# chrischoy/DeepGlobalRegistration

Measured on NVIDIA H100. Metric: scan_pairs_per_sec, higher is better.
Workload: dtype f32

## Files before the change

### deepglobalregistration_b200/csrc/spconv_ring.h

```cpp
#pragma once

#if defined(__CUDACC__)
#define DGR_RING_HD __host__ __device__ __forceinline__
#else
#define DGR_RING_HD inline
#endif

namespace spconv_ring {

constexpr int kStages = 2;
constexpr int kIdxSlots = kStages + 1;
constexpr int kMaxRun = 8;

DGR_RING_HD int stage_of(unsigned g) { return (int)(g % kStages); }
DGR_RING_HD unsigned full_parity(unsigned g) { return (g / kStages) & 1u; }
DGR_RING_HD unsigned empty_parity(unsigned g) { return (g / kStages - 1u) & 1u; }
DGR_RING_HD int idx_slot(unsigned tile) { return (int)(tile % kIdxSlots); }

constexpr int kMinWaves = 2;
DGR_RING_HD int tile_run(int n_tiles, int resident) {
  const int r = n_tiles / (kMinWaves * (resident > 0 ? resident : 1));
  return r < 1 ? 1 : (r > kMaxRun ? kMaxRun : r);
}

}
```

### deepglobalregistration_b200/csrc/spconv_tc.cu

```cuda
#include <stdlib.h>

#include "common.cuh"
#include "spconv_ring.h"
#include "tc_common.cuh"

namespace {

using namespace tc;
using namespace spconv_ring;

#define DGR_TRY_RC(expr)             \
  do {                              \
    int32_t rc__ = (expr);          \
    if (rc__ != DGR_OK) return rc__; \
  } while (0)

constexpr int kConsumerWarps = 8;
constexpr int kProducerThreads = 128;
constexpr int kThreadsTC = kConsumerWarps * 32 + kProducerThreads;
constexpr int kTileM = 128;
constexpr int kChunk = 32;
constexpr int kATileBytes = kTileM * 128;
constexpr int kGatherRows = kTileM / (kProducerThreads / 8);
static_assert(kMaxRun <= 32, "one warp lists the tiles of a run");

struct TileDesc {
  int kappa, p0, rows;
};

struct TcShared {
  unsigned long long full[kStages];
  unsigned long long empty[kStages];
  int n_run;
  TileDesc tiles[kMaxRun];
  int out_rows[kIdxSlots][kTileM];
};

constexpr bool tc_line_epilogue(int nt) { return nt >= 128; }
constexpr int kScratchLd = 40;
constexpr int kScratchBytes = 16 * kScratchLd * 4;

constexpr size_t tc_smem_bytes(int nt) {
  return sizeof(TcShared) + 1024 + (size_t)kStages * (2 * kATileBytes + 2 * nt * 128) +
         (tc_line_epilogue(nt) ? (size_t)kConsumerWarps * kScratchBytes : 0);
}

constexpr int tc_min_ctas(int nt, bool f16) { return nt >= 128 || f16 ? 1 : 2; }
constexpr int kProducerRegs = 104, kConsumerRegs = 200;

template <int NT, bool kF16, int kPasses>
__global__ void __launch_bounds__(kThreadsTC, tc_min_ctas(NT, kF16))
spconv_tc_kernel(const float* __restrict__ in_feat, int cin, const unsigned char* __restrict__ wt, int cout,
                 const int32_t* __restrict__ in_idx, const int32_t* __restrict__ out_idx,
                 const int32_t* __restrict__ kofs, const int32_t* __restrict__ tile_k,
                 const int32_t* __restrict__ tile_start, int n_tiles, int run, const float* __restrict__ amax_in,
                 const float* __restrict__ w_inv_scale, float* __restrict__ out) {
  constexpr int kCh = kF16 ? 64 : kChunk;
  constexpr int kV = kF16 ? 2 : 1;
  constexpr int kBatches = kV, kBatchRows = kGatherRows / kBatches;
  constexpr int kBTileBytes = NT * 128;
  constexpr int kStageBytes = 2 * kATileBytes + 2 * kBTileBytes;
  extern __shared__ __align__(16) unsigned char smem_dyn[];
  TcShared& sh = *reinterpret_cast<TcShared*>(smem_dyn);
  unsigned char* stage0 = reinterpret_cast<unsigned char*>(
      (reinterpret_cast<uintptr_t>(smem_dyn) + sizeof(TcShared) + 1023) & ~(uintptr_t)1023);
  const int t = threadIdx.x, warp = __shfl_sync(0xffffffffu, t >> 5, 0), lane = t & 31;
  const int n_chunks = cin / kCh;
  const uint32_t b_tile_bytes = (uint32_t)cout * 128;
  const uint32_t slab_bytes = 2 * b_tile_bytes;
  const uint32_t full0 = smem_u32(&sh.full[0]), empty0 = smem_u32(&sh.empty[0]);

  if (t == 0) {
    for (int s = 0; s < kStages; ++s) {
      mbar_init(full0 + 8 * s, kProducerThreads + 1);
      mbar_init(empty0 + 8 * s, kConsumerWarps);
    }
    asm volatile("fence.mbarrier_init.release.cluster;" ::: "memory");
  }
  if (NT > cout) {
    const int pad_pieces = (NT - cout) * 8;
    for (int i = t; i < kStages * 2 * pad_pieces; i += kThreadsTC) {
      const int tile = i / pad_pieces, e = i % pad_pieces;
      *reinterpret_cast<uint4*>(stage0 + (tile >> 1) * kStageBytes + 2 * kATileBytes + (tile & 1) * kBTileBytes +
                                (cout + (e >> 3)) * 128 + (e & 7) * 16) = make_uint4(0u, 0u, 0u, 0u);
    }
  }
  if (warp == 0) {
    const int tile = blockIdx.x * run + lane;
    TileDesc d = {0, 0, 0};
    if (lane < run && tile < n_tiles) {
      d.kappa = tile_k[tile];
      d.p0 = tile_start[tile];
      d.rows = min(kTileM, kofs[d.kappa + 1] - d.p0);
    }
    const unsigned live = __ballot_sync(0xffffffffu, d.rows > 0);
    if (d.rows > 0) sh.tiles[__popc(live & ((1u << lane) - 1u))] = d;
    if (lane == 0) sh.n_run = __popc(live);
  }
  __syncthreads();
  const int n_run = sh.n_run;
  if (n_run == 0) return;

  if (warp >= kConsumerWarps) {
    if (NT >= 128) asm volatile("setmaxnreg.dec.sync.aligned.u32 %0;" ::"n"(kProducerRegs));
    const int pt = t - kConsumerWarps * 32, piece = pt & 7, rgrp = pt >> 3;
    const uint32_t a_off = (uint32_t)(rgrp * 128 + ((piece ^ (rgrp & 7)) << 4));
    const float sx = kF16 ? f16_scale_for(__ldg(amax_in)) : 1.f;
    auto load_idx = [&](int ti, int (&src)[kGatherRows], int& oj) {
      const TileDesc d = sh.tiles[ti < n_run ? ti : 0];
      const int rows = ti < n_run ? d.rows : 0;
#pragma unroll
      for (int i = 0; i < kGatherRows; ++i) {
        const int r = i * 16 + rgrp;
        src[i] = r < rows ? __ldg(in_idx + d.p0 + r) : -1;
      }
      oj = pt < rows ? __ldg(out_idx + d.p0 + pt) : -1;
    };
    int src[kGatherRows], src_next[kGatherRows], oj, oj_next;
    float4 v[kBatchRows][kV];
    auto load_a = [&](int c, int h) {
#pragma unroll
      for (int i = 0; i < kBatchRows; ++i)
#pragma unroll
        for (int u = 0; u < kV; ++u) {
          const int row = src[h * kBatchRows + i];
          v[i][u] = row >= 0 ? __ldg(reinterpret_cast<const float4*>(in_feat + (size_t)row * cin + c * kCh +
                                                                      piece * (4 * kV) + 4 * u))
                             : make_float4(0.f, 0.f, 0.f, 0.f);
        }
    };
    load_idx(0, src, oj);
    load_idx(1, src_next, oj_next);
    load_a(0, 0);
    unsigned g = 0;
    for (int ti = 0; ti < n_run; ++ti) {
      const unsigned char* slab = wt + (size_t)sh.tiles[ti].kappa * n_chunks * slab_bytes;
      for (int c = 0; c < n_chunks; ++c, ++g) {
        const int s = stage_of(g);
        unsigned char* a_hi = stage0 + (size_t)s * kStageBytes;
        unsigned char* a_lo = a_hi + kATileBytes;
        unsigned char* b_hi = a_lo + kATileBytes;
        if (g >= kStages) mbar_wait(empty0 + 8 * s, empty_parity(g));
        if (pt == 0) {
          const unsigned char* bsrc = slab + (size_t)c * slab_bytes;
          mbar_arrive_expect_tx(full0 + 8 * s, kPasses == 3 ? slab_bytes : b_tile_bytes);
          bulk_g2s(smem_u32(b_hi), bsrc, b_tile_bytes, full0 + 8 * s);
          if (kPasses == 3) bulk_g2s(smem_u32(b_hi + kBTileBytes), bsrc + b_tile_bytes, b_tile_bytes, full0 + 8 * s);
        }
        if (c == 0) sh.out_rows[idx_slot(ti)][pt] = oj;
#pragma unroll
        for (int h = 0; h < kBatches; ++h) {
#pragma unroll
          for (int i = 0; i < kBatchRows; ++i) {
            const uint32_t off = a_off + (h * kBatchRows + i) * 2048;
            if (kF16) split_store_f16(v[i][0], v[i][kV - 1], sx, a_hi, a_lo, off);
            else split_store(v[i][0], a_hi, a_lo, off);
          }
          if (h + 1 < kBatches) {
            load_a(c, h + 1);
          } else if (c + 1 < n_chunks) {
            load_a(c + 1, 0);
          } else if (ti + 1 < n_run) {
#pragma unroll
            for (int i = 0; i < kGatherRows; ++i) src[i] = src_next[i];
            oj = oj_next;
            load_a(0, 0);
            load_idx(ti + 2, src_next, oj_next);
          }
        }
        fence_proxy_async();
        mbar_arrive(full0 + 8 * s);
      }
    }
    return;
  }

  if (NT >= 128) asm volatile("setmaxnreg.inc.sync.aligned.u32 %0;" ::"n"(kConsumerRegs));
  const int wg = warp >> 2;
  const int r0 = wg * 64 + (warp & 3) * 16 + (lane >> 2);
  const float inv = kF16 ? __ldg(w_inv_scale) / f16_scale_for(__ldg(amax_in)) : 1.f;
  auto release = [&](unsigned gq) {
    __syncwarp();
    if (lane == 0) mbar_arrive(empty0 + 8 * stage_of(gq));
  };
  unsigned g = 0;
  for (int ti = 0; ti < n_run; ++ti) {
    float acc[NT / 2];
#pragma unroll
    for (int i = 0; i < NT / 2; ++i) acc[i] = 0.f;
    for (int c = 0; c < n_chunks; ++c, ++g) {
      const uint32_t a_hi = smem_u32(stage0 + (size_t)stage_of(g) * kStageBytes);
      const uint32_t b_hi = a_hi + 2 * kATileBytes;
      mbar_wait(full0 + 8 * stage_of(g), full_parity(g));
      wgmma_fence();
      const uint32_t a0 = a_hi + wg * (kATileBytes / 2);
      mma_chunk<NT, kF16, kPasses>(acc, a0, a0 + kATileBytes, b_hi, b_hi + kBTileBytes);
      wgmma_commit();
      wgmma_wait<1>();
      if (c > 0) release(g - 1);
    }
    wgmma_wait<0>();
    fence_acc(acc);
    release(g - 1);

    const int* rows_of = sh.out_rows[idx_slot(ti)];
    if constexpr (tc_line_epilogue(NT)) {
      float* scr = reinterpret_cast<float*>(stage0 + (size_t)kStages * kStageBytes + warp * kScratchBytes);
      const int lr = lane >> 2, lc = 2 * (lane & 3);
      const int sr = lane >> 3, sc = 4 * (lane & 7);
      int js[4];
#pragma unroll
      for (int k = 0; k < 4; ++k) js[k] = rows_of[r0 - lr + sr + 4 * k];
#pragma unroll
      for (int b = 0; b < NT / 32; ++b) {
        if (32 * b >= cout) break;
#pragma unroll
        for (int q = 0; q < 4; ++q) {
          const int i = 4 * b + q;
          *reinterpret_cast<float2*>(scr + lr * kScratchLd + 8 * q + lc) =
              make_float2(acc[4 * i] * inv, acc[4 * i + 1] * inv);
          *reinterpret_cast<float2*>(scr + (lr + 8) * kScratchLd + 8 * q + lc) =
              make_float2(acc[4 * i + 2] * inv, acc[4 * i + 3] * inv);
        }
        __syncwarp();
#pragma unroll
        for (int k = 0; k < 4; ++k) {
          const float4 v = *reinterpret_cast<const float4*>(scr + (sr + 4 * k) * kScratchLd + sc);
          if (js[k] >= 0 && 32 * b + sc < cout) red_add_v4(out + (size_t)js[k] * cout + 32 * b + sc, v.x, v.y, v.z, v.w);
        }
        __syncwarp();
      }
    } else {
      const int j0 = rows_of[r0], j1 = rows_of[r0 + 8];
      float* o0 = out + (size_t)(j0 < 0 ? 0 : j0) * cout;
      float* o1 = out + (size_t)(j1 < 0 ? 0 : j1) * cout;
#pragma unroll
      for (int i = 0; i < NT / 8; ++i) {
        const int col = 8 * i + 2 * (lane & 3);
        if (col < cout) {
          if (j0 >= 0) red_add_v2(o0 + col, acc[4 * i] * inv, acc[4 * i + 1] * inv);
          if (j1 >= 0) red_add_v2(o1 + col, acc[4 * i + 2] * inv, acc[4 * i + 3] * inv);
        }
      }
    }
  }
}

template <int NT, bool kF16, int kPasses>
int tc_resident_ctas(size_t smem) {
  int dev = 0, sms = 0, per_sm = 0;
  if (cudaGetDevice(&dev) != cudaSuccess ||
      cudaDeviceGetAttribute(&sms, cudaDevAttrMultiProcessorCount, dev) != cudaSuccess ||
      cudaOccupancyMaxActiveBlocksPerMultiprocessor(&per_sm, spconv_tc_kernel<NT, kF16, kPasses>, kThreadsTC, smem) !=
          cudaSuccess)
    return 0;
  return sms * per_sm;
}

template <int NT, bool kF16, int kPasses>
int32_t launch_spconv_tc(const float* in_feat, int cin, const void* wt, int cout, const int32_t* in_idx,
                         const int32_t* out_idx, const int32_t* kofs, const int32_t* tile_k, const int32_t* tile_start,
                         int n_tiles, const float* amax_in, const float* w_inv_scale, float* out, cudaStream_t st) {
  const size_t smem = tc_smem_bytes(NT);
  DGR_ENSURE_SMEM((spconv_tc_kernel<NT, kF16, kPasses>), smem);
  static const int resident = tc_resident_ctas<NT, kF16, kPasses>(smem);
  if (resident <= 0) {
    dgr_set_error("spconv_tc_kernel does not fit the device");
    return DGR_ERR_CUDA;
  }
  const int run = tile_run(n_tiles, resident);
  spconv_tc_kernel<NT, kF16, kPasses><<<(n_tiles + run - 1) / run, kThreadsTC, smem, st>>>(
      in_feat, cin, (const unsigned char*)wt, cout, in_idx, out_idx, kofs, tile_k, tile_start, n_tiles, run, amax_in,
      w_inv_scale, out);
  dgr_note_launches(1);
  DGR_LAUNCH_CHECK();
  return DGR_OK;
}

template <bool kF16, int kPasses>
int32_t launch_spconv_tc(const float* in_feat, int cin, const void* wt, int cout, const int32_t* in_idx,
                         const int32_t* out_idx, const int32_t* kofs, const int32_t* tile_k, const int32_t* tile_start,
                         int n_tiles, const float* amax_in, const float* w_inv_scale, float* out, cudaStream_t st) {
  auto launch = cout <= 32 ? launch_spconv_tc<32, kF16, kPasses> : cout <= 64 ? launch_spconv_tc<64, kF16, kPasses>
                : cout <= 128 ? launch_spconv_tc<128, kF16, kPasses> : launch_spconv_tc<256, kF16, kPasses>;
  return launch(in_feat, cin, wt, cout, in_idx, out_idx, kofs, tile_k, tile_start, n_tiles, amax_in, w_inv_scale, out, st);
}

__global__ void pack_weight_kernel(const float* __restrict__ w, int cin, int cout, float* __restrict__ packed) {
  const int n_chunks = cin / kChunk;
  const int64_t total = (int64_t)n_chunks * cout * 8;
  const int64_t e = (int64_t)blockIdx.x * blockDim.x + threadIdx.x;
  if (e >= total) return;
  const int kappa = blockIdx.y;
  const int n = (int)(e % cout);
  const int q = (int)((e / cout) % 8);
  const int ch = (int)(e / ((int64_t)cout * 8));
  const float* src = w + ((size_t)kappa * cin + ch * kChunk + q * 4) * cout + n;
  float4 v = make_float4(src[0], src[cout], src[2 * (size_t)cout], src[3 * (size_t)cout]);
  float4 h, l;
  h.x = tf32_round(v.x); h.y = tf32_round(v.y); h.z = tf32_round(v.z); h.w = tf32_round(v.w);
  l.x = v.x - h.x; l.y = v.y - h.y; l.z = v.z - h.z; l.w = v.w - h.w;
  float* slab = packed + ((size_t)kappa * n_chunks + ch) * 2 * cout * 32;
  const int off = n * 32 + ((q ^ (n & 7)) << 2);
  *reinterpret_cast<float4*>(slab + off) = h;
  *reinterpret_cast<float4*>(slab + (size_t)cout * 32 + off) = l;
}

__global__ void absmax_kernel(const float* __restrict__ x, int64_t n, unsigned* __restrict__ out) {
  float m = 0.f;
  const int64_t n4 = n >> 2;
  for (int64_t i = (int64_t)blockIdx.x * blockDim.x + threadIdx.x; i < n4; i += (int64_t)gridDim.x * blockDim.x) {
    const float4 v = __ldg(reinterpret_cast<const float4*>(x) + i);
    m = fmaxf(fmaxf(m, fmaxf(fabsf(v.x), fabsf(v.y))), fmaxf(fabsf(v.z), fabsf(v.w)));
  }
  if (blockIdx.x == 0 && threadIdx.x < (n & 3)) m = fmaxf(m, fabsf(x[(n4 << 2) + threadIdx.x]));
#pragma unroll
  for (int d = 16; d > 0; d >>= 1) m = fmaxf(m, __shfl_xor_sync(0xffffffffu, m, d));
  if ((threadIdx.x & 31) == 0 && m > 0.f) atomicMax(out, __float_as_uint(m));
}

__global__ void pack_weight_f16_kernel(const float* __restrict__ w, int cin, int cout, const float* __restrict__ amax,
                                       unsigned char* __restrict__ packed, float* __restrict__ scale) {
  const int n_chunks = cin / 64;
  const int64_t total = (int64_t)n_chunks * cout * 8;
  const int64_t e = (int64_t)blockIdx.x * blockDim.x + threadIdx.x;
  const float sw = f16_scale_for(*amax);
  if (e == 0 && blockIdx.y == 0) scale[0] = 1.f / sw;
  if (e >= total) return;
  const int kappa = blockIdx.y;
  const int n = (int)(e % cout);
  const int q = (int)((e / cout) % 8);
  const int ch = (int)(e / ((int64_t)cout * 8));
  const float* src = w + ((size_t)kappa * cin + ch * 64 + q * 8) * cout + n;
  uint32_t h[4], l[4];
#pragma unroll
  for (int i = 0; i < 4; ++i) {
    const float x0 = src[(size_t)(2 * i) * cout] * sw, x1 = src[(size_t)(2 * i + 1) * cout] * sw;
    const __half2 hh = __floats2half2_rn(x0, x1);
    const float2 hf = __half22float2(hh);
    const __half2 ll = __floats2half2_rn(x0 - hf.x, x1 - hf.y);
    h[i] = *reinterpret_cast<const uint32_t*>(&hh);
    l[i] = *reinterpret_cast<const uint32_t*>(&ll);
  }
  unsigned char* slab = packed + ((size_t)kappa * n_chunks + ch) * 2 * cout * 128;
  const int off = n * 128 + ((q ^ (n & 7)) << 4);
  *reinterpret_cast<uint4*>(slab + off) = make_uint4(h[0], h[1], h[2], h[3]);
  *reinterpret_cast<uint4*>(slab + (size_t)cout * 128 + off) = make_uint4(l[0], l[1], l[2], l[3]);
}

}

extern "C" {

int32_t dgr_pack_weight_tf32(const float* w, int32_t K, int32_t cin, int32_t cout, float* packed, void* stream) {
  DGR_ARG_CHECK(K >= 1 && cin >= 32 && cin % 32 == 0 && cout >= 8 && cout % 8 == 0, "bad weight shape");
  DGR_ARG_CHECK(K <= 65535, "K too large");
  const int64_t per_k = (int64_t)(cin / kChunk) * cout * 8;
  dim3 grid(dgr_blocks(per_k, 256), K);
  pack_weight_kernel<<<grid, 256, 0, (cudaStream_t)stream>>>(w, cin, cout, packed);
  dgr_note_launches(1);
  DGR_LAUNCH_CHECK();
  return DGR_OK;
}


int32_t dgr_spconv_tc_supported(int32_t cin, int32_t cout) {
  return (cin >= 32 && cin % 32 == 0 && cout >= 16 && cout <= 256 && cout % 16 == 0) ? 1 : 0;
}

int32_t dgr_spconv_tc_fwd(const float* in_feat, int32_t cin, const float* weight_t, int32_t cout,
                          const int32_t* in_idx, const int32_t* out_idx, const int32_t* kofs,
                          const int32_t* tile_k, const int32_t* tile_start, int32_t n_tiles,
                          int32_t tile_rows, int32_t passes, float* out, void* stream) {
  DGR_ARG_CHECK(tile_rows == kTileM, "tile_rows must be 128");
  DGR_ARG_CHECK(dgr_spconv_tc_supported(cin, cout), "shape not supported by the tensor-core path");
  DGR_ARG_CHECK(passes == 1 || passes == 3, "passes must be 1 or 3");
  DGR_ARG_CHECK(((uintptr_t)out & 15) == 0, "out must be 16-byte aligned");
  if (n_tiles == 0) return DGR_OK;
  auto launch = passes == 3 ? launch_spconv_tc<false, 3> : launch_spconv_tc<false, 1>;
  return launch(in_feat, cin, weight_t, cout, in_idx, out_idx, kofs, tile_k, tile_start, n_tiles, nullptr, nullptr, out,
                (cudaStream_t)stream);
}

int32_t dgr_absmax_f32(const float* x, int64_t n, float* amax, void* stream) {
  cudaStream_t st = (cudaStream_t)stream;
  DGR_CUDA_CHECK(cudaMemsetAsync(amax, 0, sizeof(float), st));
  if (n <= 0) return DGR_OK;
  int dev = 0, sms = 0;
  DGR_CUDA_CHECK(cudaGetDevice(&dev));
  DGR_CUDA_CHECK(cudaDeviceGetAttribute(&sms, cudaDevAttrMultiProcessorCount, dev));
  unsigned blocks = dgr_blocks(n / 4 + 1, 256);
  if (blocks > 4u * sms) blocks = 4u * sms;
  absmax_kernel<<<blocks, 256, 0, st>>>(x, n, reinterpret_cast<unsigned*>(amax));
  dgr_note_launches(1);
  DGR_LAUNCH_CHECK();
  return DGR_OK;
}

int32_t dgr_spconv_tc_f16_supported(int32_t cin, int32_t cout) {
  return (cin >= 64 && cin % 64 == 0 && cout >= 32 && cout <= 256 && cout % 32 == 0) ? 1 : 0;
}

int32_t dgr_pack_weight_f16(const float* w, int32_t K, int32_t cin, int32_t cout, void* packed, float* scale_ws,
                            void* stream) {
  DGR_ARG_CHECK(K >= 1 && K <= 65535 && dgr_spconv_tc_f16_supported(cin, cout), "bad weight shape");
  DGR_TRY_RC(dgr_absmax_f32(w, (int64_t)K * cin * cout, scale_ws + 1, stream));
  const int64_t per_k = (int64_t)(cin / 64) * cout * 8;
  dim3 grid(dgr_blocks(per_k, 256), K);
  pack_weight_f16_kernel<<<grid, 256, 0, (cudaStream_t)stream>>>(w, cin, cout, scale_ws + 1, (unsigned char*)packed,
                                                               scale_ws);
  dgr_note_launches(1);
  DGR_LAUNCH_CHECK();
  return DGR_OK;
}

int32_t dgr_spconv_tc_f16_fwd(const float* in_feat, int32_t cin, const void* weight_h, int32_t cout,
                              const int32_t* in_idx, const int32_t* out_idx, const int32_t* kofs,
                              const int32_t* tile_k, const int32_t* tile_start, int32_t n_tiles, int32_t tile_rows,
                              const float* amax_in, const float* w_scale, float* out, void* stream) {
  DGR_ARG_CHECK(tile_rows == kTileM, "tile_rows must be 128");
  DGR_ARG_CHECK(dgr_spconv_tc_f16_supported(cin, cout), "shape not supported by the 3xFP16 path");
  DGR_ARG_CHECK(amax_in != nullptr && w_scale != nullptr, "scales missing");
  DGR_ARG_CHECK(((uintptr_t)out & 15) == 0, "out must be 16-byte aligned");
  if (n_tiles == 0) return DGR_OK;
  return launch_spconv_tc<true, 3>(in_feat, cin, weight_h, cout, in_idx, out_idx, kofs, tile_k, tile_start, n_tiles,
                                   amax_in, w_scale, out, (cudaStream_t)stream);
}

}
```

### deepglobalregistration_b200/csrc/tc_common.cuh

```cuda
#pragma once
#include <cuda_fp16.h>
#include <cuda_runtime.h>
#include <stdint.h>

#include "wgmma.cuh"

namespace tc {

__device__ __forceinline__ uint32_t smem_u32(const void* p) {
  return (uint32_t)__cvta_generic_to_shared(p);
}
__device__ __forceinline__ void mbar_init(uint32_t bar, uint32_t count) {
  asm volatile("mbarrier.init.shared::cta.b64 [%0], %1;" ::"r"(bar), "r"(count) : "memory");
}
__device__ __forceinline__ bool mbar_try_wait(uint32_t bar, uint32_t parity) {
  uint32_t ok;
  asm volatile(
      "{\n\t.reg .pred p;\n\t"
      "mbarrier.try_wait.parity.shared::cta.b64 p, [%1], %2;\n\t"
      "selp.u32 %0, 1, 0, p;\n\t}"
      : "=r"(ok)
      : "r"(bar), "r"(parity)
      : "memory");
  return ok != 0;
}
__device__ __forceinline__ void mbar_wait(uint32_t bar, uint32_t parity) {
  while (!mbar_try_wait(bar, parity)) {
  }
}
__device__ __forceinline__ void mbar_arrive(uint32_t bar) {
  asm volatile("mbarrier.arrive.shared::cta.b64 _, [%0];" ::"r"(bar) : "memory");
}
__device__ __forceinline__ void mbar_arrive_expect_tx(uint32_t bar, uint32_t bytes) {
  asm volatile("mbarrier.arrive.expect_tx.shared::cta.b64 _, [%0], %1;" ::"r"(bar), "r"(bytes) : "memory");
}
__device__ __forceinline__ void fence_proxy_async() {
  asm volatile("fence.proxy.async.shared::cta;" ::: "memory");
}
__device__ __forceinline__ void bulk_g2s(uint32_t dst_smem, const void* src, uint32_t bytes, uint32_t bar) {
  asm volatile("cp.async.bulk.shared::cluster.global.mbarrier::complete_tx::bytes [%0], [%1], %2, [%3];" ::"r"(
                   dst_smem),
               "l"(src), "r"(bytes), "r"(bar)
               : "memory");
}

__device__ __forceinline__ uint64_t wgmma_desc(uint32_t smem_addr) {
  uint64_t d = 0;
  d |= (uint64_t)((smem_addr & 0x3FFFFu) >> 4);
  d |= (uint64_t)1 << 16;
  d |= (uint64_t)(1024 >> 4) << 32;
  d |= (uint64_t)1 << 62;
  return d;
}
__device__ __forceinline__ void wgmma_fence() { asm volatile("wgmma.fence.sync.aligned;" ::: "memory"); }
__device__ __forceinline__ void wgmma_commit() { asm volatile("wgmma.commit_group.sync.aligned;" ::: "memory"); }
template <int kPending>
__device__ __forceinline__ void wgmma_wait() {
  asm volatile("wgmma.wait_group.sync.aligned %0;" ::"n"(kPending) : "memory");
}
template <int R>
__device__ __forceinline__ void fence_acc(float (&d)[R]) {
#pragma unroll
  for (int i = 0; i < R; ++i) asm volatile("" : "+f"(d[i])::"memory");
}

__device__ __forceinline__ void red_add_v2(float* addr, float a, float b) {
  asm volatile("red.global.add.v2.f32 [%0], {%1, %2};" ::"l"(addr), "f"(a), "f"(b) : "memory");
}
__device__ __forceinline__ void red_add_v4(float* addr, float a, float b, float c, float d) {
  asm volatile("red.global.add.v4.f32 [%0], {%1, %2, %3, %4};" ::"l"(addr), "f"(a), "f"(b), "f"(c), "f"(d)
               : "memory");
}
__device__ __forceinline__ float tf32_round(float x) {
  uint32_t r;
  asm("cvt.rna.tf32.f32 %0, %1;" : "=r"(r) : "f"(x));
  return __uint_as_float(r);
}

__device__ __forceinline__ void split_store(float4 v, unsigned char* hi_tile, unsigned char* lo_tile, uint32_t off) {
  float4 h, l;
  h.x = tf32_round(v.x); h.y = tf32_round(v.y); h.z = tf32_round(v.z); h.w = tf32_round(v.w);
  l.x = v.x - h.x; l.y = v.y - h.y; l.z = v.z - h.z; l.w = v.w - h.w;
  *reinterpret_cast<float4*>(hi_tile + off) = h;
  *reinterpret_cast<float4*>(lo_tile + off) = l;
}

__device__ __forceinline__ void split_store_f16(float4 a, float4 b, float sx, unsigned char* hi_tile,
                                                unsigned char* lo_tile, uint32_t off) {
  const float x[8] = {a.x * sx, a.y * sx, a.z * sx, a.w * sx, b.x * sx, b.y * sx, b.z * sx, b.w * sx};
  uint32_t h[4], l[4];
#pragma unroll
  for (int i = 0; i < 4; ++i) {
    const __half2 hh = __floats2half2_rn(x[2 * i], x[2 * i + 1]);
    const float2 hf = __half22float2(hh);
    const __half2 ll = __floats2half2_rn(x[2 * i] - hf.x, x[2 * i + 1] - hf.y);
    h[i] = *reinterpret_cast<const uint32_t*>(&hh);
    l[i] = *reinterpret_cast<const uint32_t*>(&ll);
  }
  *reinterpret_cast<uint4*>(hi_tile + off) = make_uint4(h[0], h[1], h[2], h[3]);
  *reinterpret_cast<uint4*>(lo_tile + off) = make_uint4(l[0], l[1], l[2], l[3]);
}
__device__ __forceinline__ float f16_scale_for(float amax) {
  const uint32_t b = __float_as_uint(amax);
  const int e = (int)((b >> 23) & 255u);
  if (e == 0 || e == 255) return 1.f;
  int se = 14 - (e - 127) + 127;
  se = se < 1 ? 1 : (se > 254 ? 254 : se);
  return __uint_as_float((uint32_t)se << 23);
}

template <int N, bool kF16, int kPasses>
__device__ __forceinline__ void mma_chunk(float (&d)[N / 2], uint32_t a_hi, uint32_t a_lo, uint32_t b_hi,
                                          uint32_t b_lo) {
#pragma unroll
  for (int ks = 0; ks < 4; ++ks) {
    const uint32_t ko = ks * 32;
    const uint64_t dbh = wgmma_desc(b_hi + ko);
    Wgmma<N, kF16>::mma(d, wgmma_desc(a_hi + ko), dbh);
    if (kPasses == 3) {
      Wgmma<N, kF16>::mma(d, wgmma_desc(a_lo + ko), dbh);
      Wgmma<N, kF16>::mma(d, wgmma_desc(a_hi + ko), wgmma_desc(b_lo + ko));
    }
  }
}

}
```

Measured before the change: 84.35.

## Deepen FP16 NT=256 ring to four stages with 64-byte swizzled chunks

For the FP16 path with 256 output channels, chunks shrink to 64-byte swizzled rows so four pipeline stages fit in shared memory instead of two. Warpgroup 1 is delayed by a named barrier so the two consumer warpgroups run out of phase. Runs are capped at four tiles, and weights are repacked with the matching 64-byte swizzle. This aims to hide gather and bulk-copy latency better, at the cost of more barrier round-trips and smaller WGMMA K steps per chunk.

```diff
diff --git a/deepglobalregistration_b200/csrc/spconv_ring.h b/deepglobalregistration_b200/csrc/spconv_ring.h
--- a/deepglobalregistration_b200/csrc/spconv_ring.h
+++ b/deepglobalregistration_b200/csrc/spconv_ring.h
@@ -9,18 +9,32 @@
 namespace spconv_ring {
 
 constexpr int kStages = 2;
-constexpr int kIdxSlots = kStages + 1;
+template <int S = kStages>
+constexpr int idx_slots() { return S + 1; }
+constexpr int kIdxSlots = idx_slots();
 constexpr int kMaxRun = 8;
 
-DGR_RING_HD int stage_of(unsigned g) { return (int)(g % kStages); }
-DGR_RING_HD unsigned full_parity(unsigned g) { return (g / kStages) & 1u; }
-DGR_RING_HD unsigned empty_parity(unsigned g) { return (g / kStages - 1u) & 1u; }
-DGR_RING_HD int idx_slot(unsigned tile) { return (int)(tile % kIdxSlots); }
+template <int S = kStages>
+DGR_RING_HD int stage_of(unsigned g) { return (int)(g % S); }
+template <int S = kStages>
+DGR_RING_HD unsigned full_parity(unsigned g) { return (g / S) & 1u; }
+template <int S = kStages>
+DGR_RING_HD unsigned empty_parity(unsigned g) { return (g / S - 1u) & 1u; }
+template <int S = kStages>
+DGR_RING_HD int idx_slot(unsigned tile) { return (int)(tile % idx_slots<S>()); }
+
+template <int S>
+DGR_RING_HD int consumer_lag(int n_chunks) {
+  const int l = n_chunks / 2;
+  return l < S ? l : S;
+}
 
 constexpr int kMinWaves = 2;
+constexpr int kMaxRunLagged = 4;
+template <int kCap = kMaxRun>
 DGR_RING_HD int tile_run(int n_tiles, int resident) {
   const int r = n_tiles / (kMinWaves * (resident > 0 ? resident : 1));
-  return r < 1 ? 1 : (r > kMaxRun ? kMaxRun : r);
+  return r < 1 ? 1 : (r > kCap ? kCap : r);
 }
 
 }
diff --git a/deepglobalregistration_b200/csrc/spconv_tc.cu b/deepglobalregistration_b200/csrc/spconv_tc.cu
--- a/deepglobalregistration_b200/csrc/spconv_tc.cu
+++ b/deepglobalregistration_b200/csrc/spconv_tc.cu
@@ -20,30 +20,36 @@
 constexpr int kThreadsTC = kConsumerWarps * 32 + kProducerThreads;
 constexpr int kTileM = 128;
 constexpr int kChunk = 32;
-constexpr int kATileBytes = kTileM * 128;
-constexpr int kGatherRows = kTileM / (kProducerThreads / 8);
 static_assert(kMaxRun <= 32, "one warp lists the tiles of a run");
+
+constexpr int tc_nt(int cout) { return cout <= 32 ? 32 : cout <= 64 ? 64 : cout <= 128 ? 128 : 256; }
+constexpr int tc_row_bytes(int nt, bool f16) { return f16 && nt == 256 ? 64 : 128; }
+constexpr int tc_stages(int nt, bool f16) { return 256 / tc_row_bytes(nt, f16); }
 
 struct TileDesc {
   int kappa, p0, rows;
 };
 
+template <int S>
 struct TcShared {
-  unsigned long long full[kStages];
-  unsigned long long empty[kStages];
+  unsigned long long full[S];
+  unsigned long long empty[S];
   int n_run;
   TileDesc tiles[kMaxRun];
-  int out_rows[kIdxSlots][kTileM];
+  int out_rows[idx_slots<S>()][kTileM];
 };
 
 constexpr bool tc_line_epilogue(int nt) { return nt >= 128; }
 constexpr int kScratchLd = 40;
 constexpr int kScratchBytes = 16 * kScratchLd * 4;
 
-constexpr size_t tc_smem_bytes(int nt) {
-  return sizeof(TcShared) + 1024 + (size_t)kStages * (2 * kATileBytes + 2 * nt * 128) +
-         (tc_line_epilogue(nt) ? (size_t)kConsumerWarps * kScratchBytes : 0);
-}
+template <int NT, bool kF16>
+constexpr size_t tc_smem_bytes() {
+  constexpr int S = tc_stages(NT, kF16), rb = tc_row_bytes(NT, kF16);
+  return sizeof(TcShared<S>) + 1024 + (size_t)S * (2 * kTileM * rb + 2 * NT * rb) +
+         (tc_line_epilogue(NT) ? (size_t)kConsumerWarps * kScratchBytes : 0);
+}
+static_assert(tc_smem_bytes<256, true>() <= 227 * 1024, "3xFP16 NT = 256 ring exceeds shared memory");
 
 constexpr int tc_min_ctas(int nt, bool f16) { return nt >= 128 || f16 ? 1 : 2; }
 constexpr int kProducerRegs = 104, kConsumerRegs = 200;
@@ -55,34 +61,39 @@
                  const int32_t* __restrict__ kofs, const int32_t* __restrict__ tile_k,
                  const int32_t* __restrict__ tile_start, int n_tiles, int run, const float* __restrict__ amax_in,
                  const float* __restrict__ w_inv_scale, float* __restrict__ out) {
-  constexpr int kCh = kF16 ? 64 : kChunk;
+  constexpr int kRB = tc_row_bytes(NT, kF16);
+  constexpr int S = tc_stages(NT, kF16);
+  constexpr int kCh = kF16 ? kRB / 2 : kRB / 4;
+  constexpr int kPieces = kRB / 16;
+  constexpr int kRowGroups = kProducerThreads / kPieces, kGatherRows = kTileM / kRowGroups;
   constexpr int kV = kF16 ? 2 : 1;
-  constexpr int kBatches = kV, kBatchRows = kGatherRows / kBatches;
-  constexpr int kBTileBytes = NT * 128;
+  constexpr int kBatches = kGatherRows * kV / 8, kBatchRows = kGatherRows / kBatches;
+  constexpr int kATileBytes = kTileM * kRB;
+  constexpr int kBTileBytes = NT * kRB;
   constexpr int kStageBytes = 2 * kATileBytes + 2 * kBTileBytes;
   extern __shared__ __align__(16) unsigned char smem_dyn[];
-  TcShared& sh = *reinterpret_cast<TcShared*>(smem_dyn);
+  TcShared<S>& sh = *reinterpret_cast<TcShared<S>*>(smem_dyn);
   unsigned char* stage0 = reinterpret_cast<unsigned char*>(
-      (reinterpret_cast<uintptr_t>(smem_dyn) + sizeof(TcShared) + 1023) & ~(uintptr_t)1023);
+      (reinterpret_cast<uintptr_t>(smem_dyn) + sizeof(TcShared<S>) + 1023) & ~(uintptr_t)1023);
   const int t = threadIdx.x, warp = __shfl_sync(0xffffffffu, t >> 5, 0), lane = t & 31;
   const int n_chunks = cin / kCh;
-  const uint32_t b_tile_bytes = (uint32_t)cout * 128;
+  const uint32_t b_tile_bytes = (uint32_t)cout * kRB;
   const uint32_t slab_bytes = 2 * b_tile_bytes;
   const uint32_t full0 = smem_u32(&sh.full[0]), empty0 = smem_u32(&sh.empty[0]);
 
   if (t == 0) {
-    for (int s = 0; s < kStages; ++s) {
+    for (int s = 0; s < S; ++s) {
       mbar_init(full0 + 8 * s, kProducerThreads + 1);
       mbar_init(empty0 + 8 * s, kConsumerWarps);
     }
     asm volatile("fence.mbarrier_init.release.cluster;" ::: "memory");
   }
   if (NT > cout) {
-    const int pad_pieces = (NT - cout) * 8;
-    for (int i = t; i < kStages * 2 * pad_pieces; i += kThreadsTC) {
+    const int pad_pieces = (NT - cout) * kPieces;
+    for (int i = t; i < S * 2 * pad_pieces; i += kThreadsTC) {
       const int tile = i / pad_pieces, e = i % pad_pieces;
       *reinterpret_cast<uint4*>(stage0 + (tile >> 1) * kStageBytes + 2 * kATileBytes + (tile & 1) * kBTileBytes +
-                                (cout + (e >> 3)) * 128 + (e & 7) * 16) = make_uint4(0u, 0u, 0u, 0u);
+                                (cout + e / kPieces) * kRB + (e % kPieces) * 16) = make_uint4(0u, 0u, 0u, 0u);
     }
   }
   if (warp == 0) {
@@ -103,15 +114,16 @@
 
   if (warp >= kConsumerWarps) {
     if (NT >= 128) asm volatile("setmaxnreg.dec.sync.aligned.u32 %0;" ::"n"(kProducerRegs));
-    const int pt = t - kConsumerWarps * 32, piece = pt & 7, rgrp = pt >> 3;
-    const uint32_t a_off = (uint32_t)(rgrp * 128 + ((piece ^ (rgrp & 7)) << 4));
+    constexpr int kPieceShift = kPieces == 8 ? 3 : 2;
+    const int pt = t - kConsumerWarps * 32, piece = pt & (kPieces - 1), rgrp = pt >> kPieceShift;
+    const uint32_t a_off = swizzle_offset<kRB>(rgrp, piece);
     const float sx = kF16 ? f16_scale_for(__ldg(amax_in)) : 1.f;
     auto load_idx = [&](int ti, int (&src)[kGatherRows], int& oj) {
       const TileDesc d = sh.tiles[ti < n_run ? ti : 0];
       const int rows = ti < n_run ? d.rows : 0;
 #pragma unroll
       for (int i = 0; i < kGatherRows; ++i) {
-        const int r = i * 16 + rgrp;
+        const int r = i * kRowGroups + rgrp;
         src[i] = r < rows ? __ldg(in_idx + d.p0 + r) : -1;
       }
       oj = pt < rows ? __ldg(out_idx + d.p0 + pt) : -1;
@@ -136,23 +148,23 @@
     for (int ti = 0; ti < n_run; ++ti) {
       const unsigned char* slab = wt + (size_t)sh.tiles[ti].kappa * n_chunks * slab_bytes;
       for (int c = 0; c < n_chunks; ++c, ++g) {
-        const int s = stage_of(g);
+        const int s = stage_of<S>(g);
         unsigned char* a_hi = stage0 + (size_t)s * kStageBytes;
         unsigned char* a_lo = a_hi + kATileBytes;
         unsigned char* b_hi = a_lo + kATileBytes;
-        if (g >= kStages) mbar_wait(empty0 + 8 * s, empty_parity(g));
+        if (g >= S) mbar_wait(empty0 + 8 * s, empty_parity<S>(g));
         if (pt == 0) {
           const unsigned char* bsrc = slab + (size_t)c * slab_bytes;
           mbar_arrive_expect_tx(full0 + 8 * s, kPasses == 3 ? slab_bytes : b_tile_bytes);
           bulk_g2s(smem_u32(b_hi), bsrc, b_tile_bytes, full0 + 8 * s);
           if (kPasses == 3) bulk_g2s(smem_u32(b_hi + kBTileBytes), bsrc + b_tile_bytes, b_tile_bytes, full0 + 8 * s);
         }
-        if (c == 0) sh.out_rows[idx_slot(ti)][pt] = oj;
+        if (c == 0) sh.out_rows[idx_slot<S>(ti)][pt] = oj;
 #pragma unroll
         for (int h = 0; h < kBatches; ++h) {
 #pragma unroll
           for (int i = 0; i < kBatchRows; ++i) {
-            const uint32_t off = a_off + (h * kBatchRows + i) * 2048;
+            const uint32_t off = a_off + (h * kBatchRows + i) * kRowGroups * kRB;
             if (kF16) split_store_f16(v[i][0], v[i][kV - 1], sx, a_hi, a_lo, off);
             else split_store(v[i][0], a_hi, a_lo, off);
           }
@@ -181,31 +193,34 @@
   const float inv = kF16 ? __ldg(w_inv_scale) / f16_scale_for(__ldg(amax_in)) : 1.f;
   auto release = [&](unsigned gq) {
     __syncwarp();
-    if (lane == 0) mbar_arrive(empty0 + 8 * stage_of(gq));
+    if (lane == 0) mbar_arrive(empty0 + 8 * stage_of<S>(gq));
   };
+  const int lag = S > 2 ? consumer_lag<S>(n_chunks) : 0;
+  if (lag > 0 && wg == 1) asm volatile("bar.sync 1, 256;" ::: "memory");
   unsigned g = 0;
   for (int ti = 0; ti < n_run; ++ti) {
     float acc[NT / 2];
 #pragma unroll
     for (int i = 0; i < NT / 2; ++i) acc[i] = 0.f;
     for (int c = 0; c < n_chunks; ++c, ++g) {
-      const uint32_t a_hi = smem_u32(stage0 + (size_t)stage_of(g) * kStageBytes);
+      const uint32_t a_hi = smem_u32(stage0 + (size_t)stage_of<S>(g) * kStageBytes);
       const uint32_t b_hi = a_hi + 2 * kATileBytes;
-      mbar_wait(full0 + 8 * stage_of(g), full_parity(g));
+      mbar_wait(full0 + 8 * stage_of<S>(g), full_parity<S>(g));
       wgmma_fence();
       const uint32_t a0 = a_hi + wg * (kATileBytes / 2);
-      mma_chunk<NT, kF16, kPasses>(acc, a0, a0 + kATileBytes, b_hi, b_hi + kBTileBytes);
+      mma_chunk<NT, kF16, kPasses, kRB>(acc, a0, a0 + kATileBytes, b_hi, b_hi + kBTileBytes);
       wgmma_commit();
       wgmma_wait<1>();
       if (c > 0) release(g - 1);
+      if (lag > 0 && wg == 0 && g + 1 == (unsigned)lag) asm volatile("bar.arrive 1, 256;" ::: "memory");
     }
     wgmma_wait<0>();
     fence_acc(acc);
     release(g - 1);
 
-    const int* rows_of = sh.out_rows[idx_slot(ti)];
+    const int* rows_of = sh.out_rows[idx_slot<S>(ti)];
     if constexpr (tc_line_epilogue(NT)) {
-      float* scr = reinterpret_cast<float*>(stage0 + (size_t)kStages * kStageBytes + warp * kScratchBytes);
+      float* scr = reinterpret_cast<float*>(stage0 + (size_t)S * kStageBytes + warp * kScratchBytes);
       const int lr = lane >> 2, lc = 2 * (lane & 3);
       const int sr = lane >> 3, sc = 4 * (lane & 7);
       int js[4];
@@ -261,14 +276,14 @@
 int32_t launch_spconv_tc(const float* in_feat, int cin, const void* wt, int cout, const int32_t* in_idx,
                          const int32_t* out_idx, const int32_t* kofs, const int32_t* tile_k, const int32_t* tile_start,
                          int n_tiles, const float* amax_in, const float* w_inv_scale, float* out, cudaStream_t st) {
-  const size_t smem = tc_smem_bytes(NT);
+  constexpr size_t smem = tc_smem_bytes<NT, kF16>();
   DGR_ENSURE_SMEM((spconv_tc_kernel<NT, kF16, kPasses>), smem);
   static const int resident = tc_resident_ctas<NT, kF16, kPasses>(smem);
   if (resident <= 0) {
     dgr_set_error("spconv_tc_kernel does not fit the device");
     return DGR_ERR_CUDA;
   }
-  const int run = tile_run(n_tiles, resident);
+  const int run = tile_run<(tc_stages(NT, kF16) > 2 ? kMaxRunLagged : kMaxRun)>(n_tiles, resident);
   spconv_tc_kernel<NT, kF16, kPasses><<<(n_tiles + run - 1) / run, kThreadsTC, smem, st>>>(
       in_feat, cin, (const unsigned char*)wt, cout, in_idx, out_idx, kofs, tile_k, tile_start, n_tiles, run, amax_in,
       w_inv_scale, out);
@@ -281,8 +296,9 @@
 int32_t launch_spconv_tc(const float* in_feat, int cin, const void* wt, int cout, const int32_t* in_idx,
                          const int32_t* out_idx, const int32_t* kofs, const int32_t* tile_k, const int32_t* tile_start,
                          int n_tiles, const float* amax_in, const float* w_inv_scale, float* out, cudaStream_t st) {
-  auto launch = cout <= 32 ? launch_spconv_tc<32, kF16, kPasses> : cout <= 64 ? launch_spconv_tc<64, kF16, kPasses>
-                : cout <= 128 ? launch_spconv_tc<128, kF16, kPasses> : launch_spconv_tc<256, kF16, kPasses>;
+  const int nt = tc_nt(cout);
+  auto launch = nt == 32 ? launch_spconv_tc<32, kF16, kPasses> : nt == 64 ? launch_spconv_tc<64, kF16, kPasses>
+                : nt == 128 ? launch_spconv_tc<128, kF16, kPasses> : launch_spconv_tc<256, kF16, kPasses>;
   return launch(in_feat, cin, wt, cout, in_idx, out_idx, kofs, tile_k, tile_start, n_tiles, amax_in, w_inv_scale, out, st);
 }
 
@@ -319,19 +335,21 @@
   if ((threadIdx.x & 31) == 0 && m > 0.f) atomicMax(out, __float_as_uint(m));
 }
 
+template <int kRowBytes>
 __global__ void pack_weight_f16_kernel(const float* __restrict__ w, int cin, int cout, const float* __restrict__ amax,
                                        unsigned char* __restrict__ packed, float* __restrict__ scale) {
-  const int n_chunks = cin / 64;
-  const int64_t total = (int64_t)n_chunks * cout * 8;
+  constexpr int kCh = kRowBytes / 2, kPieces = kRowBytes / 16;
+  const int n_chunks = cin / kCh;
+  const int64_t total = (int64_t)n_chunks * cout * kPieces;
   const int64_t e = (int64_t)blockIdx.x * blockDim.x + threadIdx.x;
   const float sw = f16_scale_for(*amax);
   if (e == 0 && blockIdx.y == 0) scale[0] = 1.f / sw;
   if (e >= total) return;
   const int kappa = blockIdx.y;
   const int n = (int)(e % cout);
-  const int q = (int)((e / cout) % 8);
-  const int ch = (int)(e / ((int64_t)cout * 8));
-  const float* src = w + ((size_t)kappa * cin + ch * 64 + q * 8) * cout + n;
+  const int q = (int)((e / cout) % kPieces);
+  const int ch = (int)(e / ((int64_t)cout * kPieces));
+  const float* src = w + ((size_t)kappa * cin + ch * kCh + q * 8) * cout + n;
   uint32_t h[4], l[4];
 #pragma unroll
   for (int i = 0; i < 4; ++i) {
@@ -342,10 +360,10 @@
     h[i] = *reinterpret_cast<const uint32_t*>(&hh);
     l[i] = *reinterpret_cast<const uint32_t*>(&ll);
   }
-  unsigned char* slab = packed + ((size_t)kappa * n_chunks + ch) * 2 * cout * 128;
-  const int off = n * 128 + ((q ^ (n & 7)) << 4);
+  unsigned char* slab = packed + ((size_t)kappa * n_chunks + ch) * 2 * cout * kRowBytes;
+  const uint32_t off = swizzle_offset<kRowBytes>(n, q);
   *reinterpret_cast<uint4*>(slab + off) = make_uint4(h[0], h[1], h[2], h[3]);
-  *reinterpret_cast<uint4*>(slab + (size_t)cout * 128 + off) = make_uint4(l[0], l[1], l[2], l[3]);
+  *reinterpret_cast<uint4*>(slab + (size_t)cout * kRowBytes + off) = make_uint4(l[0], l[1], l[2], l[3]);
 }
 
 }
@@ -405,10 +423,10 @@
                             void* stream) {
   DGR_ARG_CHECK(K >= 1 && K <= 65535 && dgr_spconv_tc_f16_supported(cin, cout), "bad weight shape");
   DGR_TRY_RC(dgr_absmax_f32(w, (int64_t)K * cin * cout, scale_ws + 1, stream));
-  const int64_t per_k = (int64_t)(cin / 64) * cout * 8;
+  const int64_t per_k = (int64_t)cin * cout / 8;
   dim3 grid(dgr_blocks(per_k, 256), K);
-  pack_weight_f16_kernel<<<grid, 256, 0, (cudaStream_t)stream>>>(w, cin, cout, scale_ws + 1, (unsigned char*)packed,
-                                                               scale_ws);
+  auto pack = tc_row_bytes(tc_nt(cout), true) == 64 ? pack_weight_f16_kernel<64> : pack_weight_f16_kernel<128>;
+  pack<<<grid, 256, 0, (cudaStream_t)stream>>>(w, cin, cout, scale_ws + 1, (unsigned char*)packed, scale_ws);
   dgr_note_launches(1);
   DGR_LAUNCH_CHECK();
   return DGR_OK;
diff --git a/deepglobalregistration_b200/csrc/tc_common.cuh b/deepglobalregistration_b200/csrc/tc_common.cuh
--- a/deepglobalregistration_b200/csrc/tc_common.cuh
+++ b/deepglobalregistration_b200/csrc/tc_common.cuh
@@ -51,6 +51,23 @@
   d |= (uint64_t)(1024 >> 4) << 32;
   d |= (uint64_t)1 << 62;
   return d;
+}
+__device__ __forceinline__ uint64_t wgmma_desc_sw64(uint32_t smem_addr) {
+  uint64_t d = 0;
+  d |= (uint64_t)((smem_addr & 0x3FFFFu) >> 4);
+  d |= (uint64_t)1 << 16;
+  d |= (uint64_t)(512 >> 4) << 32;
+  d |= (uint64_t)2 << 62;
+  return d;
+}
+template <int kRowBytes>
+__device__ __forceinline__ uint64_t wgmma_desc_rows(uint32_t smem_addr) {
+  static_assert(kRowBytes == 128 || kRowBytes == 64, "128- or 64-byte swizzle rows");
+  return kRowBytes == 128 ? wgmma_desc(smem_addr) : wgmma_desc_sw64(smem_addr);
+}
+template <int kRowBytes>
+__host__ __device__ __forceinline__ uint32_t swizzle_offset(int r, int q) {
+  return (uint32_t)(r * kRowBytes + ((q ^ (kRowBytes == 128 ? r & 7 : (r >> 1) & 3)) << 4));
 }
 __device__ __forceinline__ void wgmma_fence() { asm volatile("wgmma.fence.sync.aligned;" ::: "memory"); }
 __device__ __forceinline__ void wgmma_commit() { asm volatile("wgmma.commit_group.sync.aligned;" ::: "memory"); }
@@ -109,17 +126,17 @@
   return __uint_as_float((uint32_t)se << 23);
 }
 
-template <int N, bool kF16, int kPasses>
+template <int N, bool kF16, int kPasses, int kRowBytes = 128>
 __device__ __forceinline__ void mma_chunk(float (&d)[N / 2], uint32_t a_hi, uint32_t a_lo, uint32_t b_hi,
                                           uint32_t b_lo) {
 #pragma unroll
-  for (int ks = 0; ks < 4; ++ks) {
+  for (int ks = 0; ks < kRowBytes / 32; ++ks) {
     const uint32_t ko = ks * 32;
-    const uint64_t dbh = wgmma_desc(b_hi + ko);
-    Wgmma<N, kF16>::mma(d, wgmma_desc(a_hi + ko), dbh);
+    const uint64_t dbh = wgmma_desc_rows<kRowBytes>(b_hi + ko);
+    Wgmma<N, kF16>::mma(d, wgmma_desc_rows<kRowBytes>(a_hi + ko), dbh);
     if (kPasses == 3) {
-      Wgmma<N, kF16>::mma(d, wgmma_desc(a_lo + ko), dbh);
-      Wgmma<N, kF16>::mma(d, wgmma_desc(a_hi + ko), wgmma_desc(b_lo + ko));
+      Wgmma<N, kF16>::mma(d, wgmma_desc_rows<kRowBytes>(a_lo + ko), dbh);
+      Wgmma<N, kF16>::mma(d, wgmma_desc_rows<kRowBytes>(a_hi + ko), wgmma_desc_rows<kRowBytes>(b_lo + ko));
     }
   }
 }
```

Result: faster. 87.10 (median of 6 runs) (+3.3%).
